# kaitlyndlee/Raytracing-Programs

Measured on AMD Instinct MI355X. Metric: primary rays/sec (= pixels/sec) at 4096x4096, quadric.scene, higher is better.
Workload: dtype f32+f64

## Files before the change

include/raycast_hip.h:

```cpp
#ifndef RAYCAST_HIP_H
#define RAYCAST_HIP_H

#include <stdio.h>
#include <stdint.h>
#include <stdbool.h>
#include <stddef.h>

#ifdef __cplusplus
extern "C" {
#endif

#ifndef objects_h
#define objects_h
typedef enum { SPHERE, PLANE, QUADRIC } shape_type_t;
typedef enum { POINT, SPOTLIGHT } light_type_t;

typedef struct shape_t {
  float diffuse_color[3];
  float specular_color[3];
  float position[3];
  float reflectivity;
  float refractivity;
  float ior;
  union {
// ... 277 lines not shown
  int long_len;
  int wave_k;
  int resolve_k;
  int coop;
  int dep_fast;
  int o0;
  int phase_c_finish;
  int single_res_cus;
  int pipe_res_cus;
  int pipe_resolvers;
  int pipe_slots;
  int pipe_timing;
  int pipe_slotstreams;
  int overlap_d2h;
  int staged_d2h;
  int prefault;
  int copy_threads;
  int side_blocks;
  int comp_stream;
  int block_min;
  int pipe_inres;
  int x0;
  int resolve_clean;
  int shard_lone;
  int team_cscan;
  int pipe_order;
  int pipe_helpers;
  int patch_host;
  int share_device;
  int headb_first;
  int pipe_last_whole;
  int ssaa_fused;
  int adaptive_blocks;
} rc_tuning;
void rc_default_tuning(rc_tuning *t);
int rc_set_tuning(const rc_tuning *t);
void rc_get_tuning(rc_tuning *t);

#define RC_GROUP_ID_BYTES 128
enum { RC_XFER_AUTO = 0,
       RC_XFER_RCCL = 1,
       RC_XFER_COPY = 2     };
typedef struct rc_group rc_group;

int rc_group_unique_id(unsigned char id[RC_GROUP_ID_BYTES]);
rc_group *rc_group_create_rank(int nranks, int rank, const unsigned char id[RC_GROUP_ID_BYTES],
                               int device);
rc_group *rc_group_create_local(int nranks, const int *devices, int transport);
void rc_group_destroy(rc_group *group);
int rc_group_size(const rc_group *group);
int rc_group_transport(const rc_group *group);

int rc_render_sharded(rc_group *group, const rc_scene *scene, int width, int height,
                      const rc_options *opt, uint8_t *d_image, rc_timing *timing);

typedef struct rc_shard_stats {
  int ranks;
  double total_ms;
  double device_ms;
  double local_ms;
  double exchange_in_ms;
  double resolve_ms;
  double phase_c_ms;
  double image_ms;
  int64_t dep_pixels;
  int64_t zero_normalize;
// ... 23 lines not shown
```

raytracing-programs_amd/__init__.py:

```python
import contextlib
import ctypes
import os
import sys
import threading

import numpy as np

PKG_DIR = os.path.dirname(os.path.abspath(__file__))
LIB_DIR = os.path.join(PKG_DIR, "lib")
BIN_DIR = os.path.join(PKG_DIR, "bin")
ROOT_DIR = os.path.dirname(PKG_DIR)

MODE_PARITY = 0
MODE_FAST = 1
MODE_CUDA = 2
MODES = {"parity": MODE_PARITY, "fast": MODE_FAST, "cuda": MODE_CUDA}


class ShapeT(ctypes.Structure):
    _fields_ = [("diffuse_color", ctypes.c_float * 3), ("specular_color", ctypes.c_float * 3),
                ("position", ctypes.c_float * 3), ("reflectivity", ctypes.c_float),
                ("refractivity", ctypes.c_float), ("ior", ctypes.c_float),
                ("u", ctypes.c_float * 10), ("type", ctypes.c_int),
                ("next", ctypes.c_void_p)]
# ... 129 lines not shown
                ("image_bytes", ctypes.c_int64)]


class RcRankStats(ctypes.Structure):
    _fields_ = [("rank", ctypes.c_int), ("rows", ctypes.c_int), ("local_ms", ctypes.c_double),
                ("exchange_ms", ctypes.c_double), ("total_ms", ctypes.c_double),
                ("dep_pixels", ctypes.c_int64)]


class RcResolverStats(ctypes.Structure):
    _fields_ = [("frames", ctypes.c_int64), ("resolve_ms_min", ctypes.c_double),
                ("resolve_ms_max", ctypes.c_double), ("resolve_ms_mean", ctypes.c_double),
                ("grid", ctypes.c_int32), ("res_cus", ctypes.c_int32),
                ("wg_per_cu", ctypes.c_int32), ("wg_per_cu_max", ctypes.c_int32),
                ("regs", ctypes.c_int32), ("scratch_bytes", ctypes.c_int32),
                ("lds_bytes", ctypes.c_int32), ("team_blocks", ctypes.c_int32),
                ("scan_rounds_max", ctypes.c_int32), ("cscan_rounds_max", ctypes.c_int32),
                ("resolve_rounds_max", ctypes.c_int32), ("pad", ctypes.c_int32),
                ("spin_wait_us_max", ctypes.c_double * 4),
                ("clock_mhz_min", ctypes.c_int32), ("clock_mhz_max", ctypes.c_int32)]


TUNING_FIELDS = ["side", "split_shade", "resolve_shared", "resolve_lds_kb", "resolve_grid",
                 "team_blocks", "helpers", "hand_run", "long_len", "wave_k", "resolve_k", "coop",
                 "dep_fast", "o0", "phase_c_finish", "single_res_cus", "pipe_res_cus",
                 "pipe_resolvers", "pipe_slots", "pipe_timing", "pipe_slotstreams", "overlap_d2h",
                 "staged_d2h", "prefault", "copy_threads", "side_blocks", "comp_stream",
                 "block_min", "pipe_inres", "x0", "resolve_clean",
                 "shard_lone", "team_cscan", "pipe_order", "pipe_helpers", "patch_host",
                 "share_device", "headb_first", "pipe_last_whole", "ssaa_fused",
                 "adaptive_blocks"]


class RcTuning(ctypes.Structure):
    _fields_ = [(n, ctypes.c_int) for n in TUNING_FIELDS]


assert ctypes.sizeof(ShapeT) == 104 and ctypes.sizeof(LightT) == 72

HIP_EXPORTS = ["raycast", "rc_default_options", "rc_scene_create", "rc_scene_destroy",
               "rc_scene_parity_defined", "rc_render", "rc_render_device", "rc_last_kernel_ms",
               "rc_profile_begin", "rc_profile_end", "rc_version", "rc_frame_submit",
               "rc_frames_wait", "rc_pipe_reset", "rc_group_unique_id", "rc_group_create_rank",
               "rc_group_create_local", "rc_group_destroy", "rc_group_size",
               "rc_group_transport", "rc_render_sharded", "rc_group_last_stats",
               "rc_default_tuning", "rc_set_tuning", "rc_get_tuning", "rc_lone_frames_check",
               "rc_debug_inject_error", "rc_group_debug_bound", "rc_resolver_stats_get",
               "rc_group_rank_stats", "rc_debug_scatter_selftest", "rc_adaptive_stats_get",
               "rc_adaptive_phase_ms", "rc_render_rates", "rc_render_rates_device",
               "rc_rate_stats_get", "rc_rate_phase_ms", "rc_filter_box", "rc_filter_tent",
               "rc_filter_check", "rc_filter_env", "rc_render_filtered",
               "rc_render_filtered_device", "rc_filter_image_device", "rc_filter_phase_ms",
               "rc_pattern_builtin", "rc_pattern_check", "rc_pattern_env", "rc_render_pattern",
               "rc_render_pattern_device", "rc_pattern_stats_get", "rc_pattern_phase_ms",
               "rc_sample_seq_builtin", "rc_sample_seq_check", "rc_accum_pass_device",
               "rc_accum_resolve_device", "rc_render_accum", "rc_accum_stats_get",
               "rc_accum_phase_ms", "rc_window_check", "rc_window_env", "rc_render_window",
               "rc_render_window_device", "rc_accum_pass_window_device"]
FRONT_EXPORTS = ["add_new_sphere", "add_new_plane", "add_new_quadric", "free_shape_list",
                 "free_light_list", "add_new_spot_light", "add_new_point_light", "parse_json",
                 "set_to_black", "ppm_WriteOutP3", "ppm_clamp"]

_libs = {}


def _load(name):
    if name not in _libs:
        path = os.path.join(LIB_DIR, name)
# ... 227 lines not shown
        with _PACK_LOCK:
            if self._packed is None:
                h = hip_lib().rc_scene_create(ctypes.byref(self.js))
                if not h:
                    raise RuntimeError("rc_scene_create failed")
                self._packed = h
            return self._packed

    def parity_defined(self):
        return bool(hip_lib().rc_scene_parity_defined(self.packed()))

    def close(self):
        if self._packed is not None:
            hip_lib().rc_scene_destroy(self._packed)
            self._packed = None
        lib = front_lib()
        if self.js.shapes_list:
            lib.free_shape_list(ctypes.cast(self.js.shapes_list, ctypes.c_void_p))
            self.js.shapes_list = None
        if self.js.lights_list:
            lib.free_light_list(ctypes.cast(self.js.lights_list, ctypes.c_void_p))
            self.js.lights_list = None

    def __del__(self):
        try:
            self.close()
        except Exception:
            pass


def get_tuning(default=False):
    t = RcTuning()
    (hip_lib().rc_default_tuning if default else hip_lib().rc_get_tuning)(ctypes.byref(t))
    return {n: getattr(t, n) for n in TUNING_FIELDS}


def set_tuning(**fields):
    cur = get_tuning()
    unknown = set(fields) - set(cur)
    if unknown:
        raise KeyError(f"unknown tuning fields {sorted(unknown)}")
    cur.update(fields)
    t = RcTuning(**cur)
    if hip_lib().rc_set_tuning(ctypes.byref(t)) != 0:
        raise ValueError(f"rc_set_tuning rejected {fields}")


class tuned:

    def __init__(self, **fields):
        self.fields = fields

    def __enter__(self):
        self.saved = get_tuning()
        set_tuning(**self.fields)
        return self

    def __exit__(self, *exc):
        set_tuning(**self.saved)
        return False


def ssaa_adaptive(s, t):
    return int(s) | (int(t) << 8)


def ssaa_factor(v):
# ... 852 lines not shown
```

raytracing-programs_amd/csrc/rc_api.hip:

```cpp
#include <hip/hip_ext.h>
#include <hip/hip_runtime.h>

#include <algorithm>
#include <atomic>
#include <chrono>
#include <cmath>
#include <condition_variable>
#include <cstdio>
#include <cstdlib>
#include <cstring>
#include <functional>
#include <initializer_list>
#include <memory>
#include <mutex>
#include <random>
#include <string>
#include <thread>
#include <vector>

#include "raycast_hip.h"
#include "rc_kernels.h"
#include "rc_runtime.h"
#include "rc_scene.h"

// ... 8 lines not shown
  rc_tuning t;
  t.side = 3;
  t.split_shade = 0;
  t.resolve_shared = 0;
  t.resolve_lds_kb = 0;
  t.resolve_grid = 0;
  t.team_blocks = -1;
  t.helpers = 16;
  t.hand_run = 128;
  t.long_len = 32768;
  t.wave_k = 2;
  t.resolve_k = 1;
  t.coop = 1;
  t.dep_fast = 1;
  t.o0 = 1;
  t.phase_c_finish = 0;
  t.single_res_cus = 0;
  t.pipe_res_cus = 0;
  t.pipe_resolvers = 2;
  t.pipe_slots = 4;
  t.pipe_timing = 1;
  t.pipe_slotstreams = 0;
  t.overlap_d2h = 1;
  t.staged_d2h = 1;
  t.prefault = 1;
  t.copy_threads = 8;
  t.side_blocks = 0;
  t.comp_stream = 2;
  t.pipe_inres = 0;
  t.x0 = 1;
  t.resolve_clean = 1;
  t.shard_lone = 1;
  t.team_cscan = 1;
  t.pipe_order = 0;
  t.pipe_helpers = 4;
  t.patch_host = 2;
  t.block_min = 3000;
  t.share_device = 0;
  t.headb_first = 24;
  t.pipe_last_whole = 1;
  t.ssaa_fused = 1;
  t.adaptive_blocks = 0;
  return t;
}
rc_tuning g_tune = default_tuning();
std::mutex g_tune_mu;
rc_tuning tune() {
  std::lock_guard<std::mutex> lk(g_tune_mu);
  return g_tune;
}
double g_last_kernel_ms = 0.0;
std::atomic<int> g_pool_threads{-1};
std::atomic<int> g_inject{-1};
int take_inject() {
  int v = g_inject.load();
  while (v >= 0 && !g_inject.compare_exchange_weak(v, v - 1)) {
  }
  return v == 0 ? 1 : 0;
}

const char* spin_site(int code) {
  static const char* site[] = {"", "team granule", "phase-C carry-in", "helper queue",
                               "injected (rc_debug_inject_error)"};
  return code >= 1 && code <= 4 ? site[code] : "?";
}

int FrameLog::enqueue(const void* team, hipStream_t st) {
  if (!ring) {
    HIP_TRY(hipHostMalloc((void**)&ring, kRing * sizeof(Entry), hipHostMallocDefault));
    for (int i = 0; i < kRing; ++i) ring[i].code = kPending;
  }
  if (head - tail >= kRing) {
    HIP_TRY(hipDeviceSynchronize());
    if (drain() < 0) return -1;
  }
// ... 498 lines not shown
using namespace rcrt;


extern "C" {

const char* rc_version(void) { return RC_VERSION; }

void rc_default_tuning(rc_tuning* t) {
  if (t) *t = default_tuning();
}

void rc_get_tuning(rc_tuning* t) {
  if (t) *t = tune();
}

int rc_set_tuning(const rc_tuning* t) {
  if (!t) return -1;
  auto in = [](int v, int lo, int hi) { return v >= lo && v <= hi; };
  const bool ok =
      in(t->side, 0, 4) && in(t->split_shade, 0, 1) && in(t->resolve_shared, 0, 1) &&
      in(t->resolve_lds_kb, 0, 152) && (t->resolve_grid == 0 || in(t->resolve_grid, 8, 1 << 16)) &&
      in(t->team_blocks, -1, 256) && in(t->helpers, 0, rc::kDenseSlots) &&
      in(t->hand_run, 1, 1 << 30) && in(t->long_len, 64, 1 << 30) && in(t->wave_k, 1, 64) &&
      in(t->resolve_k, 1, 64) && in(t->coop, 0, 1) && in(t->dep_fast, 0, 1) && in(t->o0, 0, 1) &&
      in(t->phase_c_finish, 0, 1) && in(t->single_res_cus, 0, 1 << 16) &&
      in(t->pipe_res_cus, 0, 1 << 16) && in(t->pipe_resolvers, 1, 4) && in(t->pipe_slots, 1, 8) &&
      in(t->pipe_timing, 0, 1) && in(t->pipe_slotstreams, 0, 1) && in(t->overlap_d2h, 0, 1) &&
      in(t->staged_d2h, 0, 1) && in(t->prefault, 0, 1) && in(t->copy_threads, 1, 32) &&
      in(t->comp_stream, 0, 2) && in(t->side_blocks, 0, 1 << 16) &&
      in(t->block_min, 0, 1 << 30) && in(t->pipe_inres, 0, 2) && in(t->x0, 0, 1) &&
      in(t->resolve_clean, 1, 64) && in(t->shard_lone, 0, 1) && in(t->team_cscan, 0, 1) &&
      in(t->pipe_order, 0, 4) && in(t->pipe_helpers, 0, rc::kDenseSlots) &&
      in(t->patch_host, 0, 2) && in(t->share_device, 0, 1) && in(t->headb_first, 0, 1 << 16) && in(t->pipe_last_whole, 0, 1) &&
      in(t->ssaa_fused, 0, 1) && in(t->adaptive_blocks, 0, 4096) &&
      !(t->split_shade && !t->side);
  if (!ok) {
    std::fprintf(stderr, "Error: rc_set_tuning: a field is out of range\n");
    return -1;
  }
  const int pool = g_pool_threads.load();
  if (pool >= 0 && t->copy_threads != pool)
    std::fprintf(stderr, "Warning: rc_set_tuning: copy_threads is fixed at the host pool's "
                 "first use (%d threads); the new value is ignored\n", pool);
  for (auto& c : g_ctx) {
    if (!c.pipe.init) continue;
    if (t->pipe_resolvers != c.pipe.built_lanes || t->pipe_slots != c.pipe.built_slots ||
        t->pipe_res_cus != c.pipe.built_res || (t->pipe_timing != 0) != c.pipe.rt_on ||
        (t->pipe_slotstreams == 0) != c.pipe.fifo || t->pipe_order != c.pipe.built_order) {
      std::fprintf(stderr, "Warning: rc_set_tuning: the pipe_* fields take effect when device "
                   "%d's frame pipeline is rebuilt (rc_pipe_reset)\n", c.device);
      break;
    }
  }
  std::lock_guard<std::mutex> lk(g_tune_mu);
  g_tune = *t;
  return 0;
}

double rc_last_kernel_ms(void) { return g_last_kernel_ms; }

void rc_default_options(rc_options* opt, int use_env) {
  opt->max_recursion = 7;
  opt->mode = RC_MODE_PARITY;
  opt->num_gpus = 1;
  opt->device = 0;
  opt->ssaa = 1;
  if (!use_env) return;
// ... 59 lines not shown
namespace rcrt {

int upload_scene(FrameBufs& b, hipStream_t stream, const rc_scene* s, rc::LaunchScene& ls) {
  const rc_packed_header* h = s->img;
  if (b.scene_src != h) {
    if (b.scene.ensure((size_t)h->bytes)) return -1;
    HIP_TRY(hipMemcpyAsync(b.scene.p, h, (size_t)h->bytes, hipMemcpyHostToDevice, stream));
    b.scene_src = h;
  }
  const char* base = (const char*)b.scene.p;
  ls.shapes = (const rc_shape*)(base + h->off_shapes);
  ls.lights = (const rc_light*)(base + h->off_lights);
  ls.pairs = (const rc_shade_pair*)(base + h->off_pairs);
  ls.n = h->n;
  ls.m = h->m;
  ls.cam_w = h->cam_w;
  ls.cam_h = h->cam_h;
  ls.refl_mask = 0;
  ls.has_quadric = 0;
  ls.o0_ok = h->o0_ok && tune().o0;
  const rc_shape* hs = (const rc_shape*)((const char*)h + h->off_shapes);
  for (int k = 0; k < h->n && k < 64; ++k)
    if (hs[k].refl > 0.0f) ls.refl_mask |= 1ull << k;
  bool cross = false;
  for (int k = 0; k < h->n; ++k)
    if (hs[k].type == RC_SHAPE_QUADRIC) {
      ls.has_quadric = 1;
      if (hs[k].qd != 0.0f || hs[k].qe != 0.0f || hs[k].qf != 0.0f) cross = true;
    }
  if (ls.has_quadric && !cross && tune().x0) ls.has_quadric = 2;
  ls.dep_fast = !(hs[h->n].opacity > 0.0f) && tune().dep_fast;
  for (int k = 0; k < h->n; ++k)
    if (!(std::fabs(hs[k].refl) < 1.0e5f)) ls.dep_fast = 0;
  return 0;
}

unsigned next_epoch(unsigned e) { return e + 1 >= 0x80000000u ? 1u : e + 1; }

int ensure_parity(DevCtx& c, FrameBufs& b, int W, int H, rc::ParityWork& w, int res_cus,
                  int piped_lane) {
  const size_t P = (size_t)W * H;
  if (b.cls.ensure(P) || b.wcarry.ensure(P * sizeof(float4)) ||
      b.deprec.ensure(P * rc::deprec_bytes()) ||
      b.rows.ensure((size_t)H * (rc::row_stats_bytes() + 2 * sizeof(int) +
                                 2 * sizeof(long long)) + 256) ||
      b.dep_pix.ensure(P * sizeof(long long)) || b.seg_key.ensure(P * sizeof(long long)) ||
      b.seg_start.ensure(P * sizeof(int)) ||
      b.seg_order.ensure((size_t)rc::kSegOrderMax * sizeof(int)) ||
      b.batch_state.ensure(3 * (P / 64 + 2) * sizeof(int)) ||
      b.counters.ensure(64) || b.team.ensure(rc::team_state_bytes()))
    return -1;
  if (P >= (size_t)1 << 31) return -1;
  if (b.cin.bytes < P * rc::kCinBytes) {
    if (b.cin.ensure(P * rc::kCinBytes) || hipMemset(b.cin.p, 0, P * rc::kCinBytes) != hipSuccess)
      return -1;
  }
  b.epoch = next_epoch(b.epoch);
  if (b.epoch == 1 && hipMemset(b.cin.p, 0, b.cin.bytes) != hipSuccess) return -1;
  const bool piped = piped_lane >= 0 ? piped_lane != 0 : res_cus != c.cus;
  const rc_tuning tu = tune();
  const int one_per_cu = tu.resolve_shared ? 0 : 1;
  int lds = !one_per_cu ? 0 : piped ? 56 * 1024 : 96 * 1024;
  if (tu.resolve_lds_kb > 0) lds = tu.resolve_lds_kb * 1024;
  int slot = 0;
  while (slot < DevCtx::kResCache && c.res_lds[slot] != lds && c.res_blocks[slot]) ++slot;
  if (slot == DevCtx::kResCache) slot = 0;
// ... 280 lines not shown
    else
      HIP_TRY(rc::launch_render(ls, W, H, row0, row_step, nrows, maxrec, d_out, zc, stream,
                                opt->mode == RC_MODE_CUDA));
    if (at > 0) {
      unsigned* cnt = (unsigned*)c.aa.count.p;
      uint32_t* list = (uint32_t*)c.aa_list.p;
      if (timed) HIP_TRY(hipEventRecord(ev[2], stream));
      HIP_TRY(rc::launch_aa_mark(d_out, W, H, at, list, cnt, stream));
      if (timed) HIP_TRY(hipEventRecord(ev[3], stream));
      HIP_TRY(rc::launch_aa_refine(ls, W, H, ss, maxrec, list, cnt, d_out, zc,
                                   rc::aa_refine_blocks(W, H, ss, c.cus, tune().adaptive_blocks),
                                   stream, opt->mode == RC_MODE_CUDA));
      HIP_TRY(hipEventRecord(c.aa.done, stream));
      c.aa.valid = true;
      c.aa.rays = ss * ss;
      c.aa.pixels = (long long)W * H;
      if (timed) c.span_ev[kSpanAdaptive] = ev;
    }
    if (timed) HIP_TRY(hipEventRecord(ev[1], stream));
    return 0;
  }
  if (row0 != 0 || row_step != 1 || nrows != H) {
    std::fprintf(stderr, "Error: parity mode renders whole images only\n");
    return -1;
  }
  rc::ParityWork w{};
  int res_cus = c.cus;
  if (tune().single_res_cus > 0) res_cus = tune().single_res_cus;
  if (res_cus < 8 || res_cus > c.cus) res_cus = c.cus;
  if (ensure_parity(c, c.fb, W, H, w, res_cus, 0)) {
    std::fprintf(stderr, "Error: out of device memory for the parity workspace\n");
    return -1;
  }
  if (w.split_shade) ls.dep_fast = 0;
  if (maxrec < 3) w.inres = 0;
  w.patch = patch;
  w.inject = take_inject();
  HIP_TRY(rc::launch_parity(ls, W, H, maxrec, d_out, w, zc, stream, timed ? ev + 1 : nullptr));
  return c.lone_log.enqueue(w.team, stream);
}

int report_spin_error(const FrameBufs& b, const char* where) {
  int e[4] = {0, 0, 0, 0};
  if (hipMemcpy(e, b.team.p, sizeof e, hipMemcpyDeviceToHost) != hipSuccess) return -1;
  if (!e[0]) return 0;
  int dq[3] = {0, 0, 0}, cnt[16] = {};
  (void)hipMemcpy(dq, (const char*)b.team.p + rc::team_dq_offset(), sizeof dq,
                  hipMemcpyDeviceToHost);
  (void)hipMemcpy(cnt, b.counters.p, sizeof cnt, hipMemcpyDeviceToHost);
  std::fprintf(stderr,
               "Error: parity resolver hand-off timed out (code %d: %s; %s) at workgroup %d, "
               "detail %d/%d; segments %d, DEP entries %d, resolver census %d, helper queue "
               "prod %d claim %d finished %d, side workgroups go %d gave-up %d\n",
               e[0], spin_site(e[0]), where, e[1], e[2], e[3], cnt[0],
               cnt[2], cnt[5], dq[0], dq[1], dq[2], cnt[12], cnt[13]);
  if (e[0] == 1) {
    const int nb = rc::team_slot_bufs(), nt = rc::team_slot_blocks();
    std::vector<unsigned long long> sl((size_t)nb * nt * 4);
    if (hipMemcpy(sl.data(), (const char*)b.team.p + rc::team_slot_offset(),
                  sl.size() * sizeof(unsigned long long), hipMemcpyDeviceToHost) == hipSuccess) {
      std::vector<int> last(nt, 0);
      for (int q = 0; q < nb; ++q)
        for (int k = 0; k < nt; ++k) {
          int r = 1 << 30;
          for (int g = 0; g < 4; ++g)
            r = std::min(r, (int)(unsigned)(sl[((size_t)q * nt + k) * 4 + g] >> 32));
          last[k] = std::max(last[k], r);
// ... 359 lines not shown
  if (p.slots < p.lanes + 1) p.slots = p.lanes + 1;
  if (p.slots > Pipe::kSlots) p.slots = Pipe::kSlots;
  p.rt_on = tu.pipe_timing != 0;
  p.fifo = tu.pipe_slotstreams == 0;
  res = res / (8 * p.lanes) * (8 * p.lanes);
  if (res < 16 * p.lanes) res = 16 * p.lanes;
  if (res > c.cus - 16) res = (c.cus - 16) / (8 * p.lanes) * (8 * p.lanes);
  const int words = (c.cus + 31) / 32;
  std::vector<uint32_t> ma(words, 0), mb(words, 0);
  for (int i = 0; i < c.cus; ++i) (i < res ? ma : mb)[i / 32] |= 1u << (i % 32);
  const bool comp = tu.comp_stream == 1 || (tu.comp_stream == 2 && pixels >= (32ll << 20));
  auto mk_res = [&]() -> int {
    for (int r = 0; r < p.lanes; ++r) {
      HIP_TRY(hipExtStreamCreateWithCUMask(&p.res[r], (uint32_t)words, ma.data()));
      if (r < 2 && comp) {
        int lo = 0, hi = 0;
        HIP_TRY(hipDeviceGetStreamPriorityRange(&lo, &hi));
        HIP_TRY(hipStreamCreateWithPriority(&p.comp[r], hipStreamNonBlocking, hi));
      }
    }
    return 0;
  };
  auto mk_pc = [&]() -> int {
    for (int r = 0; r < p.lanes; ++r)
      if (p.fifo) HIP_TRY(hipExtStreamCreateWithCUMask(&p.pc[r], (uint32_t)words, mb.data()));
    return 0;
  };
  auto mk_pix = [&]() -> int {
    for (int k = 0; k < p.slots; ++k)
      if (!p.fifo || k < 2)
        HIP_TRY(hipExtStreamCreateWithCUMask(&p.pix[k], (uint32_t)words, mb.data()));
    return 0;
  };
  if (tu.pipe_order == 0) {
    for (int r = 0; r < p.lanes; ++r) {
      HIP_TRY(hipExtStreamCreateWithCUMask(&p.res[r], (uint32_t)words, ma.data()));
      if (r < 2 && comp) {
        int lo = 0, hi = 0;
        HIP_TRY(hipDeviceGetStreamPriorityRange(&lo, &hi));
        HIP_TRY(hipStreamCreateWithPriority(&p.comp[r], hipStreamNonBlocking, hi));
      }
      if (p.fifo) HIP_TRY(hipExtStreamCreateWithCUMask(&p.pc[r], (uint32_t)words, mb.data()));
    }
    if (mk_pix()) return -1;
  } else if (tu.pipe_order == 1) {
    if (mk_res() || mk_pix() || mk_pc()) return -1;
  } else if (tu.pipe_order == 3 && p.fifo && p.lanes == 2) {
    if (mk_res()) return -1;
    HIP_TRY(hipExtStreamCreateWithCUMask(&p.pix[0], (uint32_t)words, mb.data()));
    HIP_TRY(hipExtStreamCreateWithCUMask(&p.pc[0], (uint32_t)words, mb.data()));
    for (int r = 0; r < 2; ++r)
      HIP_TRY(hipExtStreamCreateWithCUMask(&p.spare[r], (uint32_t)words, ma.data()));
    HIP_TRY(hipExtStreamCreateWithCUMask(&p.pix[1], (uint32_t)words, mb.data()));
    HIP_TRY(hipExtStreamCreateWithCUMask(&p.pc[1], (uint32_t)words, mb.data()));
  } else if (tu.pipe_order == 4 && p.fifo && p.lanes == 2) {
    for (int r = 0; r < 2; ++r)
      HIP_TRY(hipExtStreamCreateWithCUMask(&p.res[r], (uint32_t)words, ma.data()));
    HIP_TRY(hipExtStreamCreateWithCUMask(&p.pc[0], (uint32_t)words, mb.data()));
    p.pc[1] = p.pc[0];
    p.pc_shared = true;
    HIP_TRY(hipExtStreamCreateWithCUMask(&p.pix[0], (uint32_t)words, mb.data()));
    for (int r = 0; r < 2; ++r)
      HIP_TRY(hipExtStreamCreateWithCUMask(&p.spare[r], (uint32_t)words, ma.data()));
    HIP_TRY(hipExtStreamCreateWithCUMask(&p.pix[1], (uint32_t)words, mb.data()));
  } else {
    if (tu.pipe_order >= 3)
      std::fprintf(stderr, "Warning: pipe_order %d needs two resolver lanes and the default "
                   "stream layout (pipe_resolvers %d, pipe_slotstreams %d): using order 2\n",
                   tu.pipe_order, p.lanes, p.fifo ? 0 : 1);
    if (mk_pix() || mk_pc() || mk_res()) return -1;
  }
  for (int k = 0; k < p.slots; ++k) {
    HIP_TRY(hipEventCreateWithFlags(&p.adone[k], hipEventDisableTiming));
    HIP_TRY(hipEventCreateWithFlags(&p.ready[k], hipEventDisableTiming));
    HIP_TRY(hipEventCreateWithFlags(&p.done[k], hipEventDisableTiming));
    HIP_TRY(hipEventCreateWithFlags(&p.cdone[k], hipEventDisableTiming));
  }
  for (auto& e : p.rt) {
    HIP_TRY(hipEventCreate(&e[0]));
    HIP_TRY(hipEventCreate(&e[1]));
  }
  p.res_cus = res;
  p.built_lanes = tu.pipe_resolvers;
  p.built_slots = tu.pipe_slots;
  p.built_res = tu.pipe_res_cus;
  p.built_order = tu.pipe_order;
  p.init = true;
  return 0;
// ... 488 lines not shown
```

raytracing-programs_amd/csrc/rc_device.hpp:

```cpp
#pragma once

#include <hip/hip_runtime.h>
#include <stdint.h>

#include "rc_scene.h"

namespace rc {

constexpr int kModeFast = 0;
constexpr int kModeParityA = 1;
constexpr int kModeParityC = 2;
constexpr int kModeClassify = 3;

constexpr uint8_t kClsIdent = 0;
constexpr uint8_t kClsWriter = 1;
constexpr uint8_t kClsDep = 2;

struct Scene {
  const rc_shape* __restrict__ shapes;
  const rc_light* __restrict__ lights;
  const rc_shade_pair* __restrict__ pairs;
  const rc_shape* lshapes;
  const rc_shade_pair* lpairs;
  int n, m;
  unsigned long long refl_mask;
  int has_quadric;
  int o0_ok;
  int dep_fast;
};

__device__ __forceinline__ bool reflective(const Scene& sc, int obj) {
  if (sc.n <= 64) return (sc.refl_mask >> obj) & 1ull;
  return sc.lshapes[obj].refl > 0.0f;
}

struct Cam {
  double hx, hy;
  float pw, ph;
};

struct V3 {
  float x, y, z;
};

__device__ __forceinline__ V3 v3(float x, float y, float z) { return V3{x, y, z}; }

__device__ __forceinline__ float dot(V3 a, V3 b) {
  float s = a.x * b.x;
  s = s + a.y * b.y;
  return s + a.z * b.z;
}
__device__ __forceinline__ V3 sub(V3 a, V3 b) { return v3(a.x - b.x, a.y - b.y, a.z - b.z); }

#ifndef RC_NRDIV
#define RC_NRDIV 1
#endif
__device__ __forceinline__ double recip_nr(double d) {
  double y = __builtin_amdgcn_rcp(d);
  double e = __builtin_fma(-d, y, 1.0);
  y = __builtin_fma(y, e, y);
  e = __builtin_fma(-d, y, 1.0);
// ... 630 lines not shown
    }
    const V3 col = shade(sc, i >= 0 ? i : sc.n, C, N, D, zero_events);
    out.x = out.x + col.x * T;
    out.y = out.y + col.y * T;
    out.z = out.z + col.z * T;
    T = T * sc.lshapes[obj].refl;
    O = C;
    S = i;
  }
  const V3 k = dep_pcol(rp);
  return v3(out.x + k.x, out.y + k.y, out.z + k.z);
}

__device__ __forceinline__ V3 carry_path(const Scene& sc, const DepRec& r, int maxrec, V3 c,
                                         int& zero_events, bool& hit) {
  V3 D = v3(r.ax, r.ay, r.az), N = v3(r.n0x, r.n0y, r.n0z), C = c;
  int obj = r.obj0, S = -1;
  hit = false;
  for (int lvl = 2; lvl < maxrec; ++lvl) {
    if (!reflective(sc, obj)) break;
    if (lvl > 2) D = normalize(reflect(D, N), zero_events);
    float t;
    const int i = nearest(sc, C, D, S, t);
    if (i >= 0) {
      V3 P;
      hit_frame(sc, i, C, D, t, P, N, zero_events);
      C = P;
      obj = i;
      hit = true;
    }
    S = i;
  }
  return C;
}

}

namespace rc {

struct LaneShape {
  rc_shape s;
  bool has;
};

template <int CTRL>
__device__ __forceinline__ int dpp_i(int v) {
  return __builtin_amdgcn_update_dpp(v, v, CTRL, 0xF, 0xF, false);
}
template <int CTRL>
__device__ __forceinline__ float dpp_f(float v) {
  return __int_as_float(__builtin_amdgcn_update_dpp(__float_as_int(v), __float_as_int(v), CTRL,
                                                    0xF, 0xF, false));
}
constexpr int kDppXor1 = 0xB1;
constexpr int kDppXor2 = 0x4E;
constexpr int kDppHalfMirror = 0x141;
constexpr int kDppRor8 = 0x128;

__device__ __forceinline__ void argmin_step(float& t, int& k, float t2, int k2) {
  if (t2 < t || (t2 == t && k2 < k)) {
    t = t2;
    k = k2;
  }
}

__device__ __forceinline__ int group_argmin(float& t, int k, int G) {
// ... 305 lines not shown
```

raytracing-programs_amd/csrc/rc_kernels.h:

```cpp
#pragma once

#include <hip/hip_runtime.h>
#include <stddef.h>
#include <stdint.h>

#include "rc_scene.h"

namespace rc {

struct LaunchScene {
  const rc_shape* shapes;
  const rc_light* lights;
  const rc_shade_pair* pairs;
  int n, m;
  float cam_w, cam_h;
  unsigned long long refl_mask;
  int has_quadric;
  int o0_ok;
  int dep_fast;
};

struct ParityWork {
  uint8_t* cls;
  float4* wcarry;
  void* deprec;
  void* row_stats;
  int* row_off;
  int* row_soff;
  long long* row_prevw;
  long long* row_prevd;
  long long* dep_pix;
  long long* seg_key;
  int* seg_start;
  void* cin;
  int* counters;
  int* batch_state;
  int* batch_cnt;
  int* batch_rq;
  hipStream_t side;
  hipEvent_t fork, join;
  int side_blocks;
  int side_lds;
  int split_shade;
  unsigned epoch;
  int* seg_order;
  void* team;
  int resolve_blocks;
  int resolve_lds;
  int team_blocks;
  int helpers;
  int hand_run;
  int long_len;
// ... 162 lines not shown
```

raytracing-programs_amd/csrc/rc_kernels.hip:

```cpp
#include <hip/hip_runtime.h>

#include <cstdio>
#include <cstdlib>
#include <type_traits>

#include "rc_cudasem.hpp"
#include "rc_device.hpp"
#include "rc_kernels.h"
#include "rc_pixel.hpp"

#ifndef RC_EXP_NODEPW
#define RC_EXP_NODEPW 0
#endif
#ifndef RC_X0_PHASE_C
#define RC_X0_PHASE_C 0
#endif
#ifndef RC_X0_RESOLVE
#define RC_X0_RESOLVE 0
#endif

namespace rc {

__device__ __forceinline__ void store_dep(uint8_t* __restrict__ out, uint32_t* __restrict__ patch,
                                          unsigned tag, long long p, int j, V3 c) {
// ... 451 lines not shown
          const int idx = idx0 + __popcll(md & lt);
          dep_pix[idx] = base + x;
          if (st) {
            const int si = s0 + __popcll(ms & lt);
            seg_start[si] = idx;
            seg_key[si] = kw;
          }
        }
        idx0 += __popcll(md);
        s0 += __popcll(ms);
        ld = base + x0 + hi_bit(md);
      }
      if (mw) lw = base + x0 + hi_bit(mw);
    }
    __syncthreads();
  }
}

#ifndef RC_HANDOFF_DIAG
#define RC_HANDOFF_DIAG 0
#endif
#ifndef RC_DIAG
#define RC_DIAG 0
#endif
#ifndef RC_TEAM_CSCAN
#define RC_TEAM_CSCAN 1
#endif
#ifndef RC_RES_GLOBAL_SCAN
#define RC_RES_GLOBAL_SCAN 0
#endif
constexpr int kResolveBlock = 256;
constexpr int kTeamMax = 256;
constexpr int kLdsShapes = kLdsShapesMax;

__device__ __forceinline__ bool same_bits(V3 a, V3 b) {
  return __float_as_uint(a.x) == __float_as_uint(b.x) &&
         __float_as_uint(a.y) == __float_as_uint(b.y) &&
         __float_as_uint(a.z) == __float_as_uint(b.z);
}

__device__ __forceinline__ V3 seg_init_carry(const long long* __restrict__ seg_key,
                                             const float4* __restrict__ wcarry, int s) {
  const long long key = seg_key[s];
  if (key < 0) return v3(0.0f, 0.0f, 0.0f);
  const float4 k4 = wcarry[key];
  return v3(k4.x, k4.y, k4.z);
}

__device__ __forceinline__ DepRec rec_at(const DepLine* __restrict__ deprec,
                                         const long long* __restrict__ dep_pix, int j) {
  return deprec[dep_pix[j]].r;
}

__device__ __forceinline__ DepRec shfl_rec(const DepRec& r, int src) {
  DepRec o;
  o.ax = __shfl(r.ax, src, 64);
  o.ay = __shfl(r.ay, src, 64);
  o.az = __shfl(r.az, src, 64);
  o.n0x = __shfl(r.n0x, src, 64);
  o.n0y = __shfl(r.n0y, src, 64);
  o.n0z = __shfl(r.n0z, src, 64);
  o.obj0 = __shfl(r.obj0, src, 64);
  o.pad = 0;
  o.bx = __shfl(r.bx, src, 64);
  o.by = __shfl(r.by, src, 64);
  o.bz = __shfl(r.bz, src, 64);
  o.pad2 = 0;
  return o;
}

struct WinStats {
  int lane, coop, changers;
// ... 1565 lines not shown
  const int ntiles = ((W + 7) >> 3) * ((H + 7) >> 3);
  while (tiles) {
    const int t = wave_ticket(&counters[7]);
    if (t >= ntiles) break;
    shade_tile(sc, cam, W, H, maxrec, t, cls, out, zero);
    if ((threadIdx.x & 63) == 0) atomicAdd(&counters[10], 1);
  }
  if (rq)
    phase_c_ready(sc, cam, W, maxrec, dep_pix, deprec, cin, counters, batch_state, rq,
                  out, patch, ts, tag, zero, nullptr);
  phase_c_passes(sc, cam, W, maxrec, dep_pix, deprec, cin, counters, batch_state, out, patch, ts, tag, false,
                 zero);
  flush_events(zero, zcount);
}

#ifndef RC_CHUNK
#define RC_CHUNK 1024
#endif
constexpr int kChunk = RC_CHUNK;

template <bool kStage, bool kFast>
__global__ void __launch_bounds__(kBlock) __attribute__((amdgpu_waves_per_eu(RC_FINISH_WAVES))) k_dep_chunks(
    Scene sc, Cam cam, int W, int row0, int row_step, int maxrec,
    const long long* __restrict__ dep_pix,
    const DepLine* __restrict__ deprec, CinG* __restrict__ cin,
    const int* __restrict__ counters, uint8_t* __restrict__ out, uint32_t* __restrict__ patch,
    unsigned long long* __restrict__ zcount, TeamState* __restrict__ ts, unsigned tag,
    int limit) {
  if (!RC_X0_PHASE_C) sc.has_quadric = sc.has_quadric != 0;
  __shared__ StageBuf<kStage> stage;
  __shared__ int s_j[kChunk];
  __shared__ float s_c[kChunk][3];
  __shared__ int s_n;
  stage_scene<kStage>(sc, stage);
  const int ndep = counters[2] < limit ? counters[2] : limit;
  const int nchunks = (ndep + kChunk - 1) / kChunk;
  const int lane = threadIdx.x & 63, wave = threadIdx.x >> 6;
  int zero = 0;
  for (int ch = blockIdx.x; ch < nchunks; ch += gridDim.x) {
    if (threadIdx.x == 0) s_n = 0;
    __syncthreads();
    for (int bb = wave; bb < kChunk / 64; bb += kBlock / 64) {
      const int b = ch * (kChunk / 64) + bb;
      if (b * 64 >= ndep) break;
      const int j = b * 64 + lane;
      V3 c = v3(0.0f, 0.0f, 0.0f);
      bool hit = true;
      (void)batch_carries(cin, ndep, b, tag, true, c, hit, ts);
      const bool in = j < ndep;
      const bool hv = in && (!kFast || hit);
      if (in && !hv) {
        const long long p = dep_pix[j];
        store_dep(out, patch, tag, p, j, dep_pcol(deprec + p));
      }
      const unsigned long long m = __ballot(hv);
      int base = 0;
      if (lane == 0 && m) base = atomicAdd(&s_n, __popcll(m));
      base = __shfl(base, 0, 64);
      if (hv) {
        const int q = base + __popcll(m & lanemask_lt());
        s_j[q] = j;
        s_c[q][0] = c.x;
        s_c[q][1] = c.y;
        s_c[q][2] = c.z;
      }
    }
    __syncthreads();
    const int n = s_n;
    for (int q = threadIdx.x; q < n; q += kBlock) {
      const int j = s_j[q];
      const V3 c = v3(s_c[q][0], s_c[q][1], s_c[q][2]);
      const long long p = dep_pix[j];
      V3 rgb;
      if constexpr (kFast) {
        rgb = shade_dep_cont(sc, deprec + p, maxrec, c, zero);
      } else {
        const int y = row0 + (int)(p / W) * row_step, x = (int)(p % W);
        const V3 d = primary_dir(cam, x, y, zero);
        PixelOut po;
        shoot<kModeParityC>(sc, d, maxrec, c, po, zero);
        rgb = po.rgb;
      }
      store_dep(out, patch, tag, p, j, rgb);
    }
    __syncthreads();
  }
  flush_events(zero, zcount);
}

struct ShardEntry {
  DepLine rec;
  float4 kc;
};
struct RowShard {
  int ndep, nstart, loff, pad;
  long long lastw, lastd, wfirst;
  float4 cw;
};
static_assert(sizeof(ShardEntry) == 80 && sizeof(RowShard) == 64, "wire records");

__global__ void __launch_bounds__(256) k_shard_pack(
// ... 443 lines not shown
```

raytracing-programs_amd/csrc/rc_pixel.hpp:

```cpp
#pragma once

#include <hip/hip_runtime.h>

#include <type_traits>

#include "rc_device.hpp"
#include "rc_kernels.h"

#ifndef RC_X0_PIXEL
#define RC_X0_PIXEL 1
#endif
#ifndef RC_PHASE_A_WAVES
#define RC_PHASE_A_WAVES 4
#endif

namespace rc {

#ifndef RC_TILE_W
#define RC_TILE_W 16
#endif
#ifndef RC_TILE_STAGE
#define RC_TILE_STAGE 0
#endif
constexpr int kTileW = RC_TILE_W, kTileH = 256 / RC_TILE_W;
// ... 101 lines not shown
template <>
struct StageBuf<false> {
  int unused;
};

template <bool kStage>
__device__ __forceinline__ void stage_scene(Scene& sc, StageBuf<kStage>& buf) {
  if constexpr (kStage) {
    const int ws = (int)(sizeof(rc_shape) / 4) * (sc.n + 1);
    for (int i = threadIdx.x; i < ws; i += blockDim.x)
      ((unsigned*)buf.s.shapes)[i] = ((const unsigned*)sc.shapes)[i];
    const int wp = (int)(sizeof(rc_shade_pair) / 4) * (sc.n + 1) * sc.m;
    for (int i = threadIdx.x; i < wp; i += blockDim.x)
      ((unsigned*)buf.s.pairs)[i] = ((const unsigned*)sc.pairs)[i];
    __syncthreads();
    sc.lshapes = buf.s.shapes;
    sc.lpairs = buf.s.pairs;
  }
}

static Scene make_scene(const LaunchScene& s) {
  Scene sc;
  sc.shapes = s.shapes;
  sc.lights = s.lights;
  sc.pairs = s.pairs;
  sc.lshapes = s.shapes;
  sc.lpairs = s.pairs;
  sc.n = s.n;
  sc.m = s.m;
  sc.refl_mask = s.refl_mask;
  sc.has_quadric = s.has_quadric;
  sc.o0_ok = s.o0_ok;
  sc.dep_fast = s.dep_fast;
  return sc;
}
static bool stage_fits(const LaunchScene& s) {
  return s.n + 1 <= kStageShapes && (s.n + 1) * s.m <= kStagePairs;
}
static Cam make_cam(const LaunchScene& s, int W, int H) {
  Cam c;
  c.hx = 0.0 - (double)s.cam_w / 2.0;
  c.hy = 0.0 + (double)s.cam_h / 2.0;
  c.pw = s.cam_w / (float)W;
  c.ph = s.cam_h / (float)H;
  return c;
}

template <class Fn>
static void dispatch(bool st, Fn fn) {
  st ? fn(std::true_type{}) : fn(std::false_type{});
}
template <class Fn>
static void dispatch(bool cuda_sem, bool st, Fn fn) {
  if (cuda_sem)
    dispatch(st, [&](auto s) { fn(std::true_type{}, s); });
  else
    dispatch(st, [&](auto s) { fn(std::false_type{}, s); });
}

}
```

raytracing-programs_amd/csrc/rc_scene.h:

```cpp
#ifndef RC_SCENE_H
#define RC_SCENE_H

#include <stdint.h>

#define RC_SHAPE_SPHERE 0
#define RC_SHAPE_PLANE 1
#define RC_SHAPE_QUADRIC 2

#define RC_LIGHT_POINT 0
#define RC_LIGHT_SPOT 1

#define RC_A0_INT 0
#define RC_A0_GENERAL 1

typedef struct rc_shape {
  int32_t type;
  float refl;
  float opacity;
  float inv_r;
  float p[3];
  float r;
  float n[3];
  float qd, qe, qf;
  float qg, qh, qi, qj;
  float qa, qb, qc;
  float o0;
  double r2;
  double A, B, C;
  double pad1;
} rc_shape;

typedef struct rc_light {
  float pos[3];
  int32_t type;
  float r0, r1, r2;
  float cos_theta;
  float dir[3];
  float a0;
  int32_t a0_kind;
  int32_t a0_int;
  float pad[2];
} rc_light;

typedef struct rc_shade_pair {
  float dl[3];
  float sl[3];
// ... 26 lines not shown
```

Before: 7.193 billion.

## Add wave-uniform pinned-origin fast path for dependent reflection shading

When every active lane in a wavefront starts its dependent reflection continuation from the same origin point, the wave builds a per-wave LDS table of origin-dependent shape terms, light directions and attenuation once. It also computes all shadow tests for the shape/light pairs in parallel across lanes and packs them into a ballot mask. The intersection and shading loops then reuse those precomputed terms instead of recomputing them per lane. The pipe_order default is also changed to 4, which alters stream creation. This adds LDS per wave and a wave-level divergence check, and it only helps when many rays share the same bounce origin.

Result: faster. 7.324 billion (median of 6 runs) (+1.8%).

```diff
diff --git a/include/raycast_hip.h b/include/raycast_hip.h
--- a/include/raycast_hip.h
+++ b/include/raycast_hip.h
@@ -333,6 +333,7 @@
   int pipe_last_whole;
   int ssaa_fused;
   int adaptive_blocks;
+  int pin;
 } rc_tuning;
 void rc_default_tuning(rc_tuning *t);
 int rc_set_tuning(const rc_tuning *t);
diff --git a/raytracing-programs_amd/__init__.py b/raytracing-programs_amd/__init__.py
--- a/raytracing-programs_amd/__init__.py
+++ b/raytracing-programs_amd/__init__.py
@@ -185,8 +185,11 @@
                  "adaptive_blocks"]
 
 
+TUNING_TAIL = ["pin"]
+
+
 class RcTuning(ctypes.Structure):
-    _fields_ = [(n, ctypes.c_int) for n in TUNING_FIELDS]
+    _fields_ = [(n, ctypes.c_int) for n in TUNING_FIELDS + TUNING_TAIL]
 
 
 assert ctypes.sizeof(ShapeT) == 104 and ctypes.sizeof(LightT) == 72
@@ -480,7 +483,7 @@
 def get_tuning(default=False):
     t = RcTuning()
     (hip_lib().rc_default_tuning if default else hip_lib().rc_get_tuning)(ctypes.byref(t))
-    return {n: getattr(t, n) for n in TUNING_FIELDS}
+    return {n: getattr(t, n) for n in TUNING_FIELDS + TUNING_TAIL}
 
 
 def set_tuning(**fields):
diff --git a/raytracing-programs_amd/csrc/rc_api.hip b/raytracing-programs_amd/csrc/rc_api.hip
--- a/raytracing-programs_amd/csrc/rc_api.hip
+++ b/raytracing-programs_amd/csrc/rc_api.hip
@@ -64,7 +64,7 @@
   t.resolve_clean = 1;
   t.shard_lone = 1;
   t.team_cscan = 1;
-  t.pipe_order = 0;
+  t.pipe_order = 4;
   t.pipe_helpers = 4;
   t.patch_host = 2;
   t.block_min = 3000;
@@ -73,6 +73,7 @@
   t.pipe_last_whole = 1;
   t.ssaa_fused = 1;
   t.adaptive_blocks = 0;
+  t.pin = 1;
   return t;
 }
 rc_tuning g_tune = default_tuning();
@@ -637,7 +638,7 @@
       in(t->resolve_clean, 1, 64) && in(t->shard_lone, 0, 1) && in(t->team_cscan, 0, 1) &&
       in(t->pipe_order, 0, 4) && in(t->pipe_helpers, 0, rc::kDenseSlots) &&
       in(t->patch_host, 0, 2) && in(t->share_device, 0, 1) && in(t->headb_first, 0, 1 << 16) && in(t->pipe_last_whole, 0, 1) &&
-      in(t->ssaa_fused, 0, 1) && in(t->adaptive_blocks, 0, 4096) &&
+      in(t->ssaa_fused, 0, 1) && in(t->adaptive_blocks, 0, 4096) && in(t->pin, 0, 3) &&
       !(t->split_shade && !t->side);
   if (!ok) {
     std::fprintf(stderr, "Error: rc_set_tuning: a field is out of range\n");
@@ -763,6 +764,7 @@
   ls.dep_fast = !(hs[h->n].opacity > 0.0f) && tune().dep_fast;
   for (int k = 0; k < h->n; ++k)
     if (!(std::fabs(hs[k].refl) < 1.0e5f)) ls.dep_fast = 0;
+  ls.pin = ls.dep_fast && RC_PIN_FITS(h->n, h->m) ? (tune().pin & 1) : 0;
   return 0;
 }
 
@@ -1109,7 +1111,7 @@
     std::fprintf(stderr, "Error: out of device memory for the parity workspace\n");
     return -1;
   }
-  if (w.split_shade) ls.dep_fast = 0;
+  if (w.split_shade) ls.dep_fast = ls.pin = 0;
   if (maxrec < 3) w.inres = 0;
   w.patch = patch;
   w.inject = take_inject();
@@ -1535,7 +1537,8 @@
         HIP_TRY(hipExtStreamCreateWithCUMask(&p.pix[k], (uint32_t)words, mb.data()));
     return 0;
   };
-  if (tu.pipe_order == 0) {
+  const bool order4 = tu.pipe_order == 4 && p.fifo && p.lanes == 2 && !comp;
+  if (tu.pipe_order == 0 || (tu.pipe_order == 4 && !order4)) {
     for (int r = 0; r < p.lanes; ++r) {
       HIP_TRY(hipExtStreamCreateWithCUMask(&p.res[r], (uint32_t)words, ma.data()));
       if (r < 2 && comp) {
@@ -1556,7 +1559,7 @@
       HIP_TRY(hipExtStreamCreateWithCUMask(&p.spare[r], (uint32_t)words, ma.data()));
     HIP_TRY(hipExtStreamCreateWithCUMask(&p.pix[1], (uint32_t)words, mb.data()));
     HIP_TRY(hipExtStreamCreateWithCUMask(&p.pc[1], (uint32_t)words, mb.data()));
-  } else if (tu.pipe_order == 4 && p.fifo && p.lanes == 2) {
+  } else if (order4) {
     for (int r = 0; r < 2; ++r)
       HIP_TRY(hipExtStreamCreateWithCUMask(&p.res[r], (uint32_t)words, ma.data()));
     HIP_TRY(hipExtStreamCreateWithCUMask(&p.pc[0], (uint32_t)words, mb.data()));
diff --git a/raytracing-programs_amd/csrc/rc_device.hpp b/raytracing-programs_amd/csrc/rc_device.hpp
--- a/raytracing-programs_amd/csrc/rc_device.hpp
+++ b/raytracing-programs_amd/csrc/rc_device.hpp
@@ -27,6 +27,7 @@
   int has_quadric;
   int o0_ok;
   int dep_fast;
+  int pin;
 };
 
 __device__ __forceinline__ bool reflective(const Scene& sc, int obj) {
@@ -723,6 +724,329 @@
     S = i;
   }
   return C;
+}
+
+__device__ __forceinline__ bool same_bits(V3 a, V3 b) {
+  return __float_as_uint(a.x) == __float_as_uint(b.x) &&
+         __float_as_uint(a.y) == __float_as_uint(b.y) &&
+         __float_as_uint(a.z) == __float_as_uint(b.z);
+}
+
+constexpr int kPinShapes = RC_PIN_SHAPES;
+constexpr int kPinLights = RC_PIN_LIGHTS;
+
+struct PinShape {
+  double b[3];
+  float o;
+  float tv[3];
+  float n[3];
+  int nev;
+};
+struct PinLight {
+  float ld[3];
+  float dist, rad, ang;
+  int z;
+  int spot;
+};
+struct PinTable {
+  PinShape s[kPinShapes];
+  PinLight l[kPinLights];
+};
+
+__device__ __forceinline__ unsigned long long pin_build(const Scene& sc, V3 c, PinTable& tb) {
+  const int lane = (int)(threadIdx.x & 63);
+  if (lane < sc.n) {
+    const rc_shape& s = sc.lshapes[lane];
+    PinShape e;
+    e.b[0] = e.b[1] = e.b[2] = 0.0;
+    e.o = 0.0f;
+    e.tv[0] = e.tv[1] = e.tv[2] = 0.0f;
+    e.nev = 0;
+    V3 N = v3(0.0f, 0.0f, 0.0f);
+    const int type = s.type;
+    if (type == RC_SHAPE_SPHERE) {
+      const V3 tv = v3(c.x - s.p[0], c.y - s.p[1], c.z - s.p[2]);
+      e.tv[0] = tv.x;
+      e.tv[1] = tv.y;
+      e.tv[2] = tv.z;
+      e.o = (float)((double)dot(tv, tv) - s.r2);
+      const float inv = s.inv_r;
+      N = normalize(v3((c.x - s.p[0]) * inv, (c.y - s.p[1]) * inv, (c.z - s.p[2]) * inv), e.nev);
+    } else if (type == RC_SHAPE_PLANE) {
+      N = v3(s.n[0], s.n[1], s.n[2]);
+      e.o = dot(v3(c.x - s.p[0], c.y - s.p[1], c.z - s.p[2]), N);
+    } else if (type == RC_SHAPE_QUADRIC) {
+      double acc;
+      acc = s.A * ((double)c.x * (double)c.x);
+      acc = acc + s.B * ((double)c.y * (double)c.y);
+      acc = acc + s.C * ((double)c.z * (double)c.z);
+      if (!quad_x0(sc)) {
+        acc = acc + (double)(s.qd * c.x * c.y);
+        acc = acc + (double)(s.qe * c.x * c.z);
+        acc = acc + (double)(s.qf * c.y * c.z);
+      }
+      acc = acc + (double)(s.qg * c.x);
+      acc = acc + (double)(s.qh * c.y);
+      acc = acc + (double)(s.qi * c.z);
+      acc = acc + (double)s.qj;
+      e.o = (float)acc;
+      e.b[0] = 2.0 * s.A * (double)c.x;
+      e.b[1] = 2.0 * s.B * (double)c.y;
+      e.b[2] = 2.0 * s.C * (double)c.z;
+      double n0 = 2.0 * s.A * (double)c.x;
+      n0 = n0 + (double)(s.qd * c.y);
+      n0 = n0 + (double)(s.qe * c.z);
+      n0 = n0 + (double)s.qg;
+      double n1 = 2.0 * s.B * (double)c.y;
+      n1 = n1 + (double)(s.qd * c.x);
+      n1 = n1 + (double)(s.qf * c.z);
+      n1 = n1 + (double)s.qh;
+      double n2 = 2.0 * s.C * (double)c.z;
+      n2 = n2 + (double)(s.qe * c.x);
+      n2 = n2 + (double)(s.qf * c.y);
+      n2 = n2 + (double)s.qi;
+      N = normalize(v3((float)n0, (float)n1, (float)n2), e.nev);
+    }
+    e.n[0] = N.x;
+    e.n[1] = N.y;
+    e.n[2] = N.z;
+    tb.s[lane] = e;
+  }
+  if (lane < sc.m) {
+    const rc_light& L = sc.lights[lane];
+    V3 ld = v3(L.pos[0] - c.x, L.pos[1] - c.y, L.pos[2] - c.z);
+    const float dist = length(ld);
+    const bool z = dist == 0.0f;
+    if (!z) ld = div3(ld, dist);
+    const float lin = L.r0 + L.r1 * dist;
+    const float rad = (float)(1.0 / ((double)lin + (double)L.r2 * ((double)dist * (double)dist)));
+    float ang = 1.0f;
+    if (L.type == RC_LIGHT_SPOT) {
+      const V3 vr = v3(c.x - L.pos[0], c.y - L.pos[1], c.z - L.pos[2]);
+      const V3 v = v3(vr.x == 0.0f ? vr.x : -ld.x, vr.y == 0.0f ? vr.y : -ld.y,
+                      vr.z == 0.0f ? vr.z : -ld.z);
+      const float alpha = dot(v, v3(L.dir[0], L.dir[1], L.dir[2]));
+      if (alpha < L.cos_theta) {
+        ang = 0.0f;
+      } else if (L.a0_kind == RC_A0_INT) {
+        ang = (float)pown_dd((double)alpha, L.a0_int);
+      } else {
+        ang = (float)pow((double)alpha, (double)L.a0);
+      }
+    }
+    PinLight e;
+    e.ld[0] = ld.x;
+    e.ld[1] = ld.y;
+    e.ld[2] = ld.z;
+    e.dist = dist;
+    e.rad = rad;
+    e.ang = ang;
+    e.z = z ? 1 : 0;
+    e.spot = L.type == RC_LIGHT_SPOT ? 1 : 0;
+    tb.l[lane] = e;
+  }
+  __builtin_amdgcn_fence(__ATOMIC_RELEASE, "wavefront");
+  __builtin_amdgcn_wave_barrier();
+  __builtin_amdgcn_fence(__ATOMIC_ACQUIRE, "wavefront");
+  bool sh = false;
+  if (lane < sc.n * sc.m) {
+    const int l = lane / sc.n, k = lane - l * sc.n;
+    const PinLight& e = tb.l[l];
+    sh = shadowed(sc, c, v3(e.ld[0], e.ld[1], e.ld[2]), k);
+  }
+  return __ballot(sh);
+}
+
+__device__ __forceinline__ int nearest_pin(const Scene& sc, V3 c, V3 D, int skip,
+                                           const PinTable& tb, float& tbest) {
+  const RayK rk = ray_consts(D);
+  const bool x0 = quad_x0(sc), rej = x0 && x0_reject(c, D);
+  float best = __builtin_inff();
+  int idx = -1;
+  for (int k = 0; k < sc.n; ++k) {
+    const rc_shape& s = sc.shapes[k];
+    const PinShape& e = tb.s[k];
+    const int type = s.type;
+    float t = 0.0f;
+    bool hit = false;
+    if (type == RC_SHAPE_SPHERE) {
+      const V3 tv = v3(e.tv[0], e.tv[1], e.tv[2]);
+      const float b = 2.0f * dot(D, tv);
+      const float fac = rk.a4 * e.o;
+      const float disc = (float)__builtin_fma((double)b, (double)b, -(double)fac);
+      if (!(disc < 0.0f)) {
+        const double sq = sqrt_ns((double)disc);
+        const float t1 = pin(tquot((double)(-b) - sq, rk.den, rk.yden));
+        const float t2 = pin(tquot((double)(-b) + sq, rk.den, rk.yden));
+        t = t1 < 0.0f ? t2 : t1;
+        hit = true;
+      }
+    } else if (type == RC_SHAPE_PLANE) {
+      const float den = dot(D, v3(s.n[0], s.n[1], s.n[2]));
+      if (!(den == 0.0f)) {
+        const float tt = (-e.o) / den;
+        if (!(tt < 0.0f)) {
+          t = tt;
+          hit = true;
+        }
+      }
+    } else if (type == RC_SHAPE_QUADRIC) {
+      double acc;
+      acc = s.A * ((double)D.x * (double)D.x);
+      acc = acc + s.B * ((double)D.y * (double)D.y);
+      acc = acc + s.C * ((double)D.z * (double)D.z);
+      if (!x0) {
+        acc = acc + (double)(s.qd * D.x * D.y);
+        acc = acc + (double)(s.qe * D.x * D.z);
+        acc = acc + (double)(s.qf * D.y * D.z);
+      }
+      const float aq = (float)acc;
+      acc = e.b[0] * (double)D.x;
+      acc = acc + e.b[1] * (double)D.y;
+      acc = acc + e.b[2] * (double)D.z;
+      if (!x0) {
+        acc = acc + (double)(s.qd * (c.x * D.y + c.y * D.x));
+        acc = acc + (double)(s.qe * (c.x * D.z + c.z * D.x));
+        acc = acc + (double)(s.qf * (c.y * D.z + c.z * D.y));
+      }
+      acc = acc + (double)(s.qg * D.x);
+      acc = acc + (double)(s.qh * D.y);
+      acc = acc + (double)(s.qi * D.z);
+      const float bq = (float)acc;
+      const float cq = e.o;
+      if (!rej) {
+        if ((double)aq == 0.0) {
+          t = tquot(-1.0 * (double)cq, (double)bq, RC_NRDIV ? recip_nr((double)bq) : 0.0);
+          hit = true;
+        } else {
+          const float disc =
+              (float)__builtin_fma((double)bq, (double)bq, -(4.0 * (double)aq * (double)cq));
+          if (!((double)disc < 0.0)) {
+            const double den = 2.0 * (double)aq;
+            const double sq = sqrt_ns((double)disc);
+            const double y = RC_NRDIV ? recip_nr(den) : 0.0;
+            const float t1 = pin(tquot((double)(-bq) - sq, den, y));
+            const float t2 = pin(tquot((double)(-bq) + sq, den, y));
+            t = t1 <= 0.0f ? t2 : t1;
+            hit = true;
+          }
+        }
+      }
+      if (hit && skip != -1 && (c.z + t * D.z) < c.z) hit = false;
+    }
+    if (hit && k != skip && best > t && t > 0.0f) {
+      best = t;
+      idx = k;
+    }
+  }
+  tbest = best;
+  return idx;
+}
+
+__device__ __forceinline__ V3 shade_pin(const Scene& sc, int idx, V3 N, V3 D, const PinTable& tb,
+                                        unsigned long long shadow, int& zero_events) {
+  const rc_shape& o = sc.lshapes[idx];
+  const float opacity = o.opacity;
+  V3 out = v3(0.0f, 0.0f, 0.0f);
+  if (!(opacity > 0.0f)) return out;
+  const rc_shade_pair* pr = sc.lpairs + (size_t)idx * sc.m;
+  for (int l = 0; l < sc.m; ++l) {
+    const PinLight& L = tb.l[l];
+    const V3 ld = v3(L.ld[0], L.ld[1], L.ld[2]);
+    const bool z = L.z != 0, spot = L.spot != 0;
+    if (z) zero_events++;
+    const float rad = L.rad, ang = L.ang;
+    const float th = dot(N, ld);
+    const bool inert = th <= 0.0f && __builtin_isfinite(rad) && __builtin_isfinite(ang) &&
+                       !(z && spot);
+    if (inert) continue;
+    if ((shadow >> (l * sc.n + idx)) & 1ull) continue;
+    if (spot) zero_events += z ? 1 : 0;
+    float dr = 0.0f, dg = 0.0f, db = 0.0f, sr = 0.0f, sg = 0.0f, sb = 0.0f;
+    if (!(th <= 0.0f)) {
+      const rc_shade_pair& p = pr[l];
+      dr = p.dl[0] * th;
+      dg = p.dl[1] * th;
+      db = p.dl[2] * th;
+      const V3 view = v3(D.x * -1.0f, D.y * -1.0f, D.z * -1.0f);
+      const double angle = (double)dot(view, reflect(ld, N));
+      if (!(angle > 0.0)) {
+        const double p20 = pow20(angle);
+        sr = (float)((double)p.sl[0] * p20);
+        sg = (float)((double)p.sl[1] * p20);
+        sb = (float)((double)p.sl[2] * p20);
+      }
+    }
+    out.x = out.x + ((dr + sr) * rad) * ang;
+    out.y = out.y + ((dg + sg) * rad) * ang;
+    out.z = out.z + ((db + sb) * rad) * ang;
+  }
+  return v3(out.x * opacity, out.y * opacity, out.z * opacity);
+}
+
+__device__ __forceinline__ V3 shade_dep_cont_pin(const Scene& sc, const DepLine* __restrict__ rp,
+                                                 int maxrec, V3 c, const PinTable& tb,
+                                                 unsigned long long shadow, int& zero_events) {
+  const DepRec& r = rp->r;
+  int obj = r.obj0, S = -1;
+  const float T0 = sc.lshapes[obj].refl;
+  float T = T0 * sc.lshapes[obj].refl;
+  V3 O = c, C = c, D = v3(r.ax, r.ay, r.az), N = v3(r.n0x, r.n0y, r.n0z);
+  V3 out = v3(0.0f, 0.0f, 0.0f);
+  for (int lvl = 2; lvl < maxrec; ++lvl) {
+    if (!reflective(sc, obj)) break;
+    if (lvl > 2) D = normalize(reflect(D, N), zero_events);
+    float t;
+    int i;
+    if (__ballot(!same_bits(O, c)) == 0ull) i = nearest_pin(sc, c, D, S, tb, t);
+    else i = nearest(sc, O, D, S, t);
+    V3 col;
+    if (i >= 0) {
+      const V3 P = v3(O.x + D.x * t, O.y + D.y * t, O.z + D.z * t);
+      if (same_bits(P, c)) {
+        const PinShape& e = tb.s[i];
+        N = v3(e.n[0], e.n[1], e.n[2]);
+        zero_events += e.nev;
+        const int type = sc.lshapes[i].type;
+        if (type != RC_SHAPE_SPHERE && type != RC_SHAPE_PLANE && dot(N, D) > 0.0f)
+          N = v3(N.x * -1.0f, N.y * -1.0f, N.z * -1.0f);
+        C = P;
+        col = shade_pin(sc, i, N, D, tb, shadow, zero_events);
+      } else {
+        hit_frame(sc, i, O, D, t, C, N, zero_events);
+        col = shade(sc, i, C, N, D, zero_events);
+      }
+      obj = i;
+    } else {
+      col = shade(sc, sc.n, C, N, D, zero_events);
+    }
+    out.x = out.x + col.x * T;
+    out.y = out.y + col.y * T;
+    out.z = out.z + col.z * T;
+    T = T * sc.lshapes[obj].refl;
+    O = C;
+    S = i;
+  }
+  const V3 k = dep_pcol(rp);
+  return v3(out.x + k.x, out.y + k.y, out.z + k.z);
+}
+
+__device__ __forceinline__ V3 shade_dep_wave(const Scene& sc, const DepLine* __restrict__ rp,
+                                             int maxrec, V3 c, bool act, PinTable& tb,
+                                             int& zero_events, bool& took) {
+  const V3 c0 = v3(__uint_as_float(__builtin_amdgcn_readfirstlane(__float_as_uint(c.x))),
+                   __uint_as_float(__builtin_amdgcn_readfirstlane(__float_as_uint(c.y))),
+                   __uint_as_float(__builtin_amdgcn_readfirstlane(__float_as_uint(c.z))));
+  V3 rgb = v3(0.0f, 0.0f, 0.0f);
+  took = __ballot(act && !same_bits(c, c0)) == 0ull;
+  if (took) {
+    const unsigned long long shadow = pin_build(sc, c0, tb);
+    if (act) rgb = shade_dep_cont_pin(sc, rp, maxrec, c0, tb, shadow, zero_events);
+    __builtin_amdgcn_fence(__ATOMIC_ACQ_REL, "wavefront");
+  } else if (act) {
+    rgb = shade_dep_cont(sc, rp, maxrec, c, zero_events);
+  }
+  return rgb;
 }
 
 }
diff --git a/raytracing-programs_amd/csrc/rc_kernels.h b/raytracing-programs_amd/csrc/rc_kernels.h
--- a/raytracing-programs_amd/csrc/rc_kernels.h
+++ b/raytracing-programs_amd/csrc/rc_kernels.h
@@ -18,6 +18,7 @@
   int has_quadric;
   int o0_ok;
   int dep_fast;
+  int pin;
 };
 
 struct ParityWork {
diff --git a/raytracing-programs_amd/csrc/rc_kernels.hip b/raytracing-programs_amd/csrc/rc_kernels.hip
--- a/raytracing-programs_amd/csrc/rc_kernels.hip
+++ b/raytracing-programs_amd/csrc/rc_kernels.hip
@@ -507,12 +507,6 @@
 constexpr int kResolveBlock = 256;
 constexpr int kTeamMax = 256;
 constexpr int kLdsShapes = kLdsShapesMax;
-
-__device__ __forceinline__ bool same_bits(V3 a, V3 b) {
-  return __float_as_uint(a.x) == __float_as_uint(b.x) &&
-         __float_as_uint(a.y) == __float_as_uint(b.y) &&
-         __float_as_uint(a.z) == __float_as_uint(b.z);
-}
 
 __device__ __forceinline__ V3 seg_init_carry(const long long* __restrict__ seg_key,
                                              const float4* __restrict__ wcarry, int s) {
@@ -2144,6 +2138,7 @@
   __shared__ int s_j[kChunk];
   __shared__ float s_c[kChunk][3];
   __shared__ int s_n;
+  __shared__ PinTable s_pin[kFast ? kBlock / 64 : 1];
   stage_scene<kStage>(sc, stage);
   const int ndep = counters[2] < limit ? counters[2] : limit;
   const int nchunks = (ndep + kChunk - 1) / kChunk;
@@ -2179,6 +2174,28 @@
     }
     __syncthreads();
     const int n = s_n;
+    if constexpr (kFast) {
+      if (sc.pin) {
+        for (int q0 = __builtin_amdgcn_readfirstlane(wave) * 64; q0 < n; q0 += kBlock) {
+          const int q = q0 + lane;
+          const bool act = q < n;
+          int j = 0;
+          long long p = 0;
+          V3 c = v3(0.0f, 0.0f, 0.0f);
+          if (act) {
+            j = s_j[q];
+            c = v3(s_c[q][0], s_c[q][1], s_c[q][2]);
+            p = dep_pix[j];
+          }
+          bool took;
+          const V3 rgb = shade_dep_wave(sc, deprec + p, maxrec, c, act,
+                                        s_pin[__builtin_amdgcn_readfirstlane(wave)], zero, took);
+          if (act) store_dep(out, patch, tag, p, j, rgb);
+        }
+        __syncthreads();
+        continue;
+      }
+    }
     for (int q = threadIdx.x; q < n; q += kBlock) {
       const int j = s_j[q];
       const V3 c = v3(s_c[q][0], s_c[q][1], s_c[q][2]);
diff --git a/raytracing-programs_amd/csrc/rc_pixel.hpp b/raytracing-programs_amd/csrc/rc_pixel.hpp
--- a/raytracing-programs_amd/csrc/rc_pixel.hpp
+++ b/raytracing-programs_amd/csrc/rc_pixel.hpp
@@ -157,6 +157,7 @@
   sc.has_quadric = s.has_quadric;
   sc.o0_ok = s.o0_ok;
   sc.dep_fast = s.dep_fast;
+  sc.pin = s.pin;
   return sc;
 }
 static bool stage_fits(const LaunchScene& s) {
diff --git a/raytracing-programs_amd/csrc/rc_scene.h b/raytracing-programs_amd/csrc/rc_scene.h
--- a/raytracing-programs_amd/csrc/rc_scene.h
+++ b/raytracing-programs_amd/csrc/rc_scene.h
@@ -12,6 +12,11 @@
 
 #define RC_A0_INT 0
 #define RC_A0_GENERAL 1
+
+#define RC_PIN_SHAPES 8
+#define RC_PIN_LIGHTS 16
+#define RC_PIN_FITS(n, m) \
+  ((n) >= 1 && (n) <= RC_PIN_SHAPES && (m) <= RC_PIN_LIGHTS && (n) * (m) <= 64)
 
 typedef struct rc_shape {
   int32_t type;
```
